# WISDEM/RAFT

Measured on AMD Instinct MI355X. Metric: design-case-frequency solves/sec (whole node), higher is better.
Workload: dtype f64

## Files before the change

### raft_amd/csrc/raftx_geom.h

```cpp
#pragma once

#define MP_N 24
#define MH_N 48
#define MI_N 48

__host__ __device__ inline void derive_design_tables(const double *strips, int64_t i0, int64_t i1, double *dsv,
                                                     int *dsf) {
    int64_t s = i0;
    while (s < i1) {
        int64_t e = s + 1;
        double proj[64];
        int np = 0;
        while (e < i1 && (e - s) < 64) {
            const double *pr = strips + (size_t)(e - 1) * NF, *cr = strips + (size_t)e * NF;
            bool same = true;
            double dv[3], pj = 0.0;
            for (int j = 0; j < 3; j++) {
                same = same && (pr[RAFTX_F_Q + j] == cr[RAFTX_F_Q + j]);
                dv[j] = cr[RAFTX_F_X + j] - pr[RAFTX_F_X + j];
                pj += dv[j] * cr[RAFTX_F_Q + j];
            }
            if (!same || !(pj > 0.0) || !(fabs(pj) <= 1.797e308)) break;
            double perp2 = 0.0, scale = 1.0;
            for (int j = 0; j < 3; j++) {
// ... 79 lines not shown
    double *Ms, *Cs, *Ws;
    const double *Fz;
    double *drho;
    double rho, g;
    int nw;
    const double *k;
    int *cnt, *cntm;
    double *mpose, *mhyd;
    double *abi;
    double *mcfaux;
    cplx *cm;
    int64_t *off, *cmoff;
    double *ds;
    int *dsi;
    double *A, *Ch, *Wh, *props;
    double *M0, *C0;
    int add_mask;
    int addup_in_design;
    long long *tot;
    long long *hostOut;
    int64_t mbase, sbase, cbase;
    int *mdesign_w;
    int mgrid;
    __device__ int64_t mo(int d) const { return memberOff[d] - mbase; }
    __device__ int64_t so(int64_t m) const { return stationOff[m] - sbase; }
    __device__ int64_t co(int64_t m) const { return capOff[m] - cbase; }
};

#define GEOM_NOFMA _Pragma("clang fp contract(off)")

__device__ inline double geom_interp(double x, const double *gs, int n, int f) {
    GEOM_NOFMA
    if (x < gs[RAFTX_GS_S]) return gs[f];
    if (x > gs[(size_t)(n - 1) * RAFTX_GS_N + RAFTX_GS_S]) return gs[(size_t)(n - 1) * RAFTX_GS_N + f];
    int j = 0;
    for (int i = 0; i < n; i++)
        if (gs[(size_t)i * RAFTX_GS_N + RAFTX_GS_S] <= x) j = i;
    const double fj = gs[(size_t)j * RAFTX_GS_N + f];
    if (j == n - 1) return fj;
    const double xj = gs[(size_t)j * RAFTX_GS_N + RAFTX_GS_S];
    if (xj == x) return fj;
    const double slope = (gs[(size_t)(j + 1) * RAFTX_GS_N + f] - fj) / (gs[(size_t)(j + 1) * RAFTX_GS_N + RAFTX_GS_S] - xj);
    return slope * (x - xj) + fj;
}

struct GLocate {
// ... 358 lines not shown
    if (d == 0) { A.off[0] = 0; A.cmoff[0] = 0; }
    if (d < A.nDesign)
        for (int64_t m = A.mo(d); m < A.mo(d + 1); m++) A.mdesign_w[m] = d;
}
#define GEOM_MAX_STATIONS 1024
__device__ inline int64_t geom_member_of_thread(const GeomArgs &A) {
    const int64_t t = (int64_t)blockIdx.x * blockDim.x + threadIdx.x;
    if (A.mgrid <= 0) return t < A.nMember ? t : -1;
    const int64_t k = t / A.nDesign;
    if (k >= A.mgrid) return -1;
    const int d = (int)(t % A.nDesign);
    const int64_t m = A.mo(d) + k;
    return m < A.mo(d + 1) ? m : -1;
}
__device__ __forceinline__ void geom_load_row(const double *gs, int i, double (&r)[RAFTX_GS_N]) {
    const double2 *p = reinterpret_cast<const double2 *>(gs + (size_t)i * RAFTX_GS_N);
#pragma unroll
    for (int k = 0; k < RAFTX_GS_N / 2; k++) {
        const double2 v = p[k];
        r[2 * k] = v.x;
        r[2 * k + 1] = v.y;
    }
}
__global__ __launch_bounds__(128) void k_geom_member(GeomArgs A) {
    GEOM_NOFMA
    if (A.mgrid > 0 && A.err[2]) return;
    const int64_t m = geom_member_of_thread(A);
    if (m < 0) return;
    if (A.err[2]) {
        A.cnt[m] = 0;
        A.cntm[m] = 0;
        return;
    }
    double gm[RAFTX_GM_N];
    {
        const double2 *p = reinterpret_cast<const double2 *>(A.gm + (size_t)m * RAFTX_GM_N);
#pragma unroll
        for (int k = 0; k < RAFTX_GM_N / 2; k++) {
            const double2 v = p[k];
            gm[2 * k] = v.x;
            gm[2 * k + 1] = v.y;
        }
    }
    const int64_t so0 = A.so(m), so1 = A.so(m + 1);
    const int64_t co0 = A.capOff ? A.co(m) : 0, co1 = A.capOff ? A.co(m + 1) : 0;
    const int d = A.mdesign[m];
    const double *gs = A.gs + (size_t)so0 * RAFTX_GS_N;
    const int n = (int)(so1 - so0);
    if (n < 2 || n > GEOM_MAX_STATIONS || !(gm[RAFTX_GM_DLSMAX] > 0.0) || !(gm[RAFTX_GM_L] > 0.0)) {
        A.cnt[m] = 0;
        A.cntm[m] = 0;
        atomicCAS(A.err + 3, 0, (int)(m + 1));
        return;
    }
    if (((int)gm[RAFTX_GM_FLAGS] & RAFTX_GM_FLAG_MCF) && gm[RAFTX_GM_SHAPE] != 0.0 && !A.k) {
        A.cnt[m] = 0;
        A.cntm[m] = 0;
        atomicCAS(A.err + 3, 0, -(int)(m + 1));
        return;
    }
    double ps[6] = {0, 0, 0, 0, 0, 0};
    if (A.pose)
        for (int i = 0; i < 6; i++) ps[i] = A.pose[(size_t)d * 6 + i];
    double a[RAFTX_GS_N], b[RAFTX_GS_N];
    geom_load_row(gs, 0, b);
    const bool circ = gm[RAFTX_GM_SHAPE] != 0.0;
    const int flags = (int)gm[RAFTX_GM_FLAGS];
    double rA0[3], q0[3], nrm = 0.0;
    for (int i = 0; i < 3; i++) {
        rA0[i] = gm[RAFTX_GM_RA + i];
        q0[i] = gm[RAFTX_GM_RB + i] - gm[RAFTX_GM_RA + i];
        nrm += q0[i] * q0[i];
    }
    nrm = sqrt(nrm);
    for (int i = 0; i < 3; i++) q0[i] /= nrm;
    const double beta = atan2(q0[1], q0[0]);
    const double phi = atan2(sqrt(q0[0] * q0[0] + q0[1] * q0[1]), q0[2]);
    const double gam = gm[RAFTX_GM_GAMMA] * (M_PI / 180.0);
    const double s1 = sin(beta), c1 = cos(beta), s2 = sin(phi), c2 = cos(phi), s3 = sin(gam), c3 = cos(gam);
    const double R0[3][3] = {{c1 * c2 * c3 - s1 * s3, -c3 * s1 - c1 * c2 * s3, c1 * s2},
                             {c1 * s3 + c2 * c3 * s1, c1 * c3 - c2 * s1 * s3, s1 * s2},
                             {-c3 * s2, s2 * s3, c2}};
    const double p10[3] = {R0[0][0], R0[1][0], R0[2][0]};
    const double p20[3] = {q0[1] * p10[2] - q0[2] * p10[1], q0[2] * p10[0] - q0[0] * p10[2], q0[0] * p10[1] - q0[1] * p10[0]};
    const double sy = sin(ps[5]), cy = cos(ps[5]), sp = sin(ps[4]), cp = cos(ps[4]), sr = sin(ps[3]), cr = cos(ps[3]);
    const double Rp[3][3] = {{cy * cp, cy * sp * sr - cr * sy, sy * sr + cy * cr * sp},
                             {cp * sy, cy * cr + sy * sp * sr, cr * sy * sp - cy * sr},
                             {-sp, cp * sr, cp * cr}};
    double q[3], p1[3], p2[3], rA[3], rB[3], R[2][2];
    const double L = gm[RAFTX_GM_L];
    for (int i = 0; i < 3; i++) {
        q[i] = Rp[i][0] * q0[0] + Rp[i][1] * q0[1] + Rp[i][2] * q0[2];
        p1[i] = Rp[i][0] * p10[0] + Rp[i][1] * p10[1] + Rp[i][2] * p10[2];
        p2[i] = Rp[i][0] * p20[0] + Rp[i][1] * p20[1] + Rp[i][2] * p20[2];
        const double dsp = (Rp[i][0] - (i == 0 ? 1.0 : 0.0)) * rA0[0] + (Rp[i][1] - (i == 1 ? 1.0 : 0.0)) * rA0[1] +
                           (Rp[i][2] - (i == 2 ? 1.0 : 0.0)) * rA0[2];
        rA[i] = rA0[i] + (ps[i] + dsp);
    }
    for (int i = 0; i < 3; i++) rB[i] = rA[i] + L * q[i];
    for (int i = 0; i < 2; i++)
        for (int j = 0; j < 2; j++) R[i][j] = Rp[i][0] * R0[0][j] + Rp[i][1] * R0[1][j] + Rp[i][2] * R0[2][j];
    int wet = 0;
    if (geom_along(rA[2], rB[2], 0.0, L) < 0) wet++;
    double C[36], F[6], Vt = 0.0, rcV[3] = {0, 0, 0}, AWPm = 0.0;
    for (int i = 0; i < 36; i++) C[i] = 0.0;
    for (int i = 0; i < 6; i++) F[i] = 0.0;
    const double beta2 = atan2(q[1], q[0]), phi2 = atan2(sqrt(q[0] * q[0] + q[1] * q[1]), q[2]);
    const double cosPhi = cos(phi2), sinPhi = sin(phi2), tanPhi = tan(phi2), cosBeta = cos(beta2), sinBeta = sin(beta2);
    const double rg = A.rho * A.g;
    const bool nostatic = (flags & RAFTX_GM_FLAG_NOSTATIC) != 0;
    const double rho_shell = gm[RAFTX_GM_RHOSHELL];
    const bool trim = (A.add_mask & RAFTX_TRIM_BALLAST) != 0;
    for (int i = 1; i < n; i++) {
#pragma unroll
        for (int f = 0; f < RAFTX_GS_N; f++) a[f] = b[f];
        geom_load_row(gs, i, b);
        {
            const double lstrip = b[RAFTX_GS_S] - a[RAFTX_GS_S];
            const int cntg = geom_interval_strips(lstrip, gm[RAFTX_GM_DLSMAX]);
            for (int j = 0; j < cntg; j++) {
                double ls;
                if (lstrip > 0.0) {
                    const double dl = lstrip / cntg;
                    ls = a[RAFTX_GS_S] + dl * (0.5 + j);
                } else {
                    ls = a[RAFTX_GS_S];
                }
                if (geom_along(rA[2], rB[2], ls, L) < 0) wet++;
            }
        }
        if (nostatic) continue;
        {
            double ra[3], rb[3];
            for (int c = 0; c < 3; c++) {
                ra[c] = rA[c] + q[c] * a[RAFTX_GS_S];
// ... 47 lines not shown
                C[4 * 6 + 5] += -rg * V * (rc[1] - rA[1]);
                Vt += V;
                for (int c = 0; c < 3; c++) rcV[c] += rc[c] * V;
                AWPm = AWP;
            } else if (ra[2] <= 0 && rb[2] <= 0) {
                double V, hc;
                geom_frustum(a[RAFTX_GS_D], aD1, b[RAFTX_GS_D], bD1, circ, b[RAFTX_GS_S] - a[RAFTX_GS_S], V, hc);
                double rc[3], rr[3];
                for (int c = 0; c < 3; c++) { rc[c] = ra[c] + q[c] * hc; rr[c] = rc[c] - rA[c]; }
                const double Fz = rg * V;
                F[2] += Fz;
                F[3] += rr[1] * Fz;
                F[4] += -rr[0] * Fz;
                C[3 * 6 + 3] += rg * V * rr[2];
                C[4 * 6 + 4] += rg * V * rr[2];
                C[3 * 6 + 5] += -rg * V * rr[0];
                C[4 * 6 + 5] += -rg * V * rr[1];
                Vt += V;
                for (int c = 0; c < 3; c++) rcV[c] += rc[c] * V;
            }
        }
    }
    if (geom_along(rA[2], rB[2], b[RAFTX_GS_S], L) < 0) wet++;
    double *mh = A.mhyd + (size_t)m * MH_N, *mi = A.minert + (size_t)m * MI_N;
    if (!nostatic) {
        for (int i = 0; i < 36; i++) mh[i] = C[i];
        for (int i = 0; i < 6; i++) mh[36 + i] = F[i];
        mh[42] = Vt; mh[43] = rcV[0]; mh[44] = rcV[1]; mh[45] = rcV[2]; mh[46] = AWPm; mh[47] = 0.0;
    }
    int code = 0;
    if (!nostatic) {
        GInertia J;
        geom_inertia_init(J);
        geom_load_row(gs, 0, b);
        for (int i = 1; i < n; i++) {
#pragma unroll
            for (int f = 0; f < RAFTX_GS_N; f++) a[f] = b[f];
            geom_load_row(gs, i, b);
            geom_inertia_section(J, a, b, circ, rho_shell, trim, 0.0, rA, q, p1, p2);
        }
        const int ncap = A.capOff ? (int)(co1 - co0) : 0;
        const double *gc = A.capOff ? A.caps + (size_t)co0 * RAFTX_GC_N : nullptr;
        code = geom_inertia_caps_finish(J, gs, n, gc, ncap, circ, rho_shell, rA, q, p1, p2, A.g, mi);
    }
    double *mp = A.mpose + (size_t)m * MP_N;
    for (int i = 0; i < 3; i++) {
        mp[i] = rA0[i]; mp[3 + i] = rA[i]; mp[6 + i] = q[i]; mp[9 + i] = p1[i]; mp[12 + i] = p2[i];
    }
    mp[15] = R[0][0]; mp[16] = R[0][1]; mp[17] = R[1][0]; mp[18] = R[1][1]; mp[19] = L;
    const int wetm = ((flags & RAFTX_GM_FLAG_MCF) && circ && !(flags & RAFTX_GM_FLAG_POTMOD)) ? wet : 0;
    A.cnt[m] = wet;
    A.cntm[m] = wetm;
    if (wet) atomicAdd(reinterpret_cast<unsigned long long *>(A.off + d + 1), (unsigned long long)wet);
    if (wetm) atomicAdd(reinterpret_cast<unsigned long long *>(A.cmoff + d + 1), (unsigned long long)wetm);
    if (nostatic) {
        for (int i = 0; i < MH_N; i++) mh[i] = 0.0;
        for (int i = 0; i < MI_N; i++) mi[i] = 0.0;
        return;
    }
    if (code) {
        for (int i = 0; i < MI_N; i++) mi[i] = 0.0;
        atomicCAS(A.err, 0, (int)(m + 1));
    }
}

__global__ void k_geom_trim(GeomArgs A) {
    GEOM_NOFMA
    if (A.err[2] | A.err[3]) return;
    const int d = blockIdx.x * blockDim.x + threadIdx.x;
    if (d >= A.nDesign) return;
    double mass = A.M0[(size_t)d * 36], V = 0.0, vol = 0.0;
    for (int64_t m = A.mo(d); m < A.mo(d + 1); m++) {
        mass += A.minert[(size_t)m * MI_N + 36];
        vol += A.minert[(size_t)m * MI_N + 47];
        V += A.mhyd[(size_t)m * MH_N + 42];
    }
    if (!(vol > 0.0)) {
        A.drho[d] = 0.0;
        atomicCAS(A.err + 1, 0, d + 1);
        return;
    }
    const double sumFz = -mass * A.g + V * A.rho * A.g + (A.Fz ? A.Fz[d] : 0.0);
    A.drho[d] = sumFz / A.g / vol;
}
__global__ __launch_bounds__(128) void k_geom_reinertia(GeomArgs A) {
    GEOM_NOFMA
// ... 184 lines not shown
#endif
static_assert(GD_T % 64 == 0 && GD_T % DS_N == 0 && GD_T <= 256, "k_geom_design: whole wavefronts, a lane keeps its record field");
template <bool ABI, bool ADDUP>
__device__ __forceinline__ void geom_design_block(const GeomArgs &A, const int d, double *gd_lds, int *wcnt) {
    GEOM_NOFMA
    const int lane = threadIdx.x;
    const int64_t i0 = A.off[d], i1 = A.off[d + 1];
    const int S = (int)(i1 - i0);
    double *rec = gd_lds;
    double *pjv = rec + (size_t)S * GD_ROW, *unv = pjv + S;
    int *okv = reinterpret_cast<int *>(unv + S), *rsv = okv + S, *mfl = rsv + S;
    GEOM_PHASE_BEGIN
    {
        const int64_t m0 = A.mo(d), m1 = A.mo(d + 1);
        const int nMem = (int)(m1 - m0);
        const int64_t s0 = A.so(m0);
        const int nSta = (int)(A.so(m1) - s0);
        int *mcum = mfl + S;
        int *mbase = mcum + nSta + 2 * nMem;
        int *ssta = mbase + nMem + 1;
        double *sgm = reinterpret_cast<double *>(okv + (((int)(ssta - okv) + nMem + 2) & ~1));
        double *sgs = sgm + (size_t)nMem * GD_GM_N;
        double *smp = sgs + (size_t)nSta * RAFTX_GS_N;
        {
            const double *g0 = A.gm + (size_t)m0 * RAFTX_GM_N, *g1 = A.gs + (size_t)s0 * RAFTX_GS_N, *g2 = A.mpose + (size_t)m0 * MP_N;
            const int n0 = nMem * GD_GM_N, n01 = n0 + nSta * RAFTX_GS_N, total = n01 + nMem * GD_MP_N;
            constexpr int SU = 10;
            const int64_t so_lane = lane <= nMem ? A.so(m0 + lane) : s0;
            for (int base = 0; base < total; base += SU * GD_T) {
                double v[SU];
#pragma unroll
                for (int u = 0; u < SU; u++) {
                    const int idx = base + u * GD_T + lane;
                    const double *src;
                    if (idx < n0) {
                        const int row = idx / GD_GM_N, col = idx % GD_GM_N;
                        src = g0 + (size_t)row * RAFTX_GM_N + (col == 0 ? RAFTX_GM_DLSMAX : (col == 1 ? RAFTX_GM_SHAPE : RAFTX_GM_FLAGS));
                    } else if (idx < n01) {
                        src = g1 + (idx - n0);
                    } else {
                        const int k = idx - n01, row = k / GD_MP_N, col = k % GD_MP_N;
                        src = g2 + (size_t)row * MP_N + (col < 12 ? 3 + col : 19);
                    }
                    v[u] = idx < total ? *src : 0.0;
                }
#pragma unroll
                for (int u = 0; u < SU; u++) {
                    const int idx = base + u * GD_T + lane;
                    if (idx < total) sgm[idx] = v[u];
                }
            }
            if (lane <= nMem) mbase[lane] = ssta[lane] = (int)(so_lane - s0);
            for (int mi = lane + GD_T; mi <= nMem; mi += GD_T) mbase[mi] = ssta[mi] = (int)(A.so(m0 + mi) - s0);
        }
        __syncthreads();
        for (int u = lane; u < nSta + nMem; u += GD_T) {
            int mi = 0;
            while (mi + 1 < nMem && mbase[mi + 1] + mi + 1 <= u) mi++;
            const int sta0 = mbase[mi], n = mbase[mi + 1] - sta0, g = u - (sta0 + mi);
            int cntg = 1;
            if (g > 0 && g < n) {
                const double *gs = sgs + (size_t)sta0 * RAFTX_GS_N;
                cntg = geom_interval_strips(gs[(size_t)g * RAFTX_GS_N + RAFTX_GS_S] - gs[(size_t)(g - 1) * RAFTX_GS_N + RAFTX_GS_S],
                                            sgm[(size_t)mi * GD_GM_N]);
            }
            mcum[sta0 + 2 * mi + g + 1] = cntg;
        }
        __syncthreads();
        for (int mi = lane; mi < nMem; mi += GD_T) {
            const int n = ssta[mi + 1] - ssta[mi];
            int *cum = mcum + ssta[mi] + 2 * mi;
            int a = 0;
            cum[0] = 0;
            for (int g = 0; g <= n; g++) { a += cum[g + 1]; cum[g + 1] = a; }
            mbase[mi + 1] = a;
        }
        __syncthreads();
        if (lane == 0) {
            int a = 0;
            mbase[0] = 0;
            for (int mi = 0; mi < nMem; mi++) { a += mbase[mi + 1]; mbase[mi + 1] = a; }
        }
        __syncthreads();
        const int total = mbase[nMem];
        GEOM_PHASE(0);
        const double rho = A.rho, cdrag = sqrt(8 / M_PI);
        double rP[3] = {0, 0, 0};
        if (A.pose)
            for (int i = 0; i < 3; i++) rP[i] = A.pose[(size_t)d * 6 + i];
        int nwet = 0;
        for (int t0 = 0; t0 < total; t0 += GD_T) {
            const int t = t0 + lane;
            const bool act = t < total;
            const int tq = act ? t : 0;
            int mi = 0;
            while (mi + 1 < nMem && mbase[mi + 1] <= tq) mi++;
            const int64_t m = m0 + mi;
// ... 469 lines not shown
```

### raft_amd/csrc/raftx_hip.hip

```cpp

#include <hip/hip_runtime.h>
#include <rccl/rccl.h>
#include <dlfcn.h>

#include <algorithm>
#include <cmath>
#include <cstdint>
#include <cstdio>
#include <cstdlib>
#include <cstring>
#include <chrono>
#include <map>
#include <functional>
#include <mutex>
#include <type_traits>
#include <thread>
#include <unordered_map>
#include <vector>

#include "../../include/raftx.h"
#include "../../include/raftx_modal.h"
#include "../../include/raftx_current.h"
#include "../../include/raftx_channels.h"

// ... 635 lines not shown
struct BuildJob {
    GeomArgs A;
    std::vector<void *> tmp;
    int nDesign = 0, nw = 0;
    int64_t maxMem = 0, maxSta = 0;
    size_t nStrips = 0, nRows = 0;
    int maxS = 0;
    double *M0d = nullptr, *C0d = nullptr;
    const double *B0d = nullptr, *MBwd = nullptr;
    bool active = false;
    hipStream_t reduce_stream = nullptr;
    bool gen_deferred = false;
    size_t gen_lds = 0;
};

struct CaseSet {
    std::vector<double> key;
    DevTables T;
    std::vector<void *> allocs;
    int users = 0;
    unsigned long long stamp = 0;
};

struct VariantProg {
    int nM = 0, nSt = 0, nCap = 0, nP = 0;
    bool has_caps = false;
    double *gm = nullptr, *gs = nullptr, *gc = nullptr;
    int *stMember = nullptr, *capMember = nullptr;
    double *stFrac = nullptr, *fillFrac = nullptr, *capFrac = nullptr;
    double *endCoef = nullptr, *headCS = nullptr, *diaCoef = nullptr;
    int *endEdit = nullptr, *diaEdit = nullptr;
    std::vector<int64_t> hS, hC;
    std::vector<void *> allocs;
    int cachedN = -1;
    std::vector<int64_t> memberOff, stationOff, capOff;
};
struct VariantSrc {
    const VariantProg *prog;
    const double *params;
};

static void expand_args(const VariantProg &P, int n, double *gm_out, double *gs_out, double *gc_out, ExpandArgs &E) {
    E.n = n; E.nM = P.nM; E.nSt = P.nSt; E.nCap = P.nCap; E.nP = P.nP;
    E.gm = P.gm; E.gs = P.gs; E.gc = P.gc;
    E.stMember = P.stMember; E.capMember = P.capMember;
    E.stFrac = P.stFrac; E.fillFrac = P.fillFrac; E.capFrac = P.capFrac;
    E.endCoef = P.endCoef; E.headCS = P.headCS; E.diaCoef = P.diaCoef;
    E.endEdit = P.endEdit; E.diaEdit = P.diaEdit;
    E.gm_out = gm_out; E.gs_out = gs_out; E.gc_out = gc_out;
}

struct DenseResident {
    int nSet = 0, n = 0, nw = 0, freq_mask = 0;
    double *w = nullptr, *M = nullptr, *B = nullptr, *C = nullptr;
    std::vector<void *> allocs;
};
struct raftx_ctx {
    int device;
    hipStream_t stream;
    bool owns_stream;
    hipEvent_t ev0, ev1;
    hipEvent_t evUp, evTot, evG0, evG1, evG2, evG3, evS0, evS1, evDone;
// ... 66 lines not shown
    int comm_rank, comm_world;
    int *commFlag = nullptr;
    std::vector<raftx_ctx *> workers[RAFTX_NSLOT];
    struct SweepSlot *slots;
    VariantProg vprog;
};
struct DevOffsets {
    const int64_t *memberOff, *stationOff, *capOff;
};
struct SeaStates { int nCase, nHead, nw; const double *w, *k; double depth, rho, g; const double *zeta, *beta; };
struct BuildSource {
    const int64_t *memberOff, *stationOff, *capOff;
    const double *members, *stations, *caps;
    const double *pose, *M0, *B0, *C0, *MBw, *Fz_moor, *k;
    double rho, g;
    int nw, add_mask;
    DevOffsets dOff{nullptr, nullptr, nullptr};
    const double *k_dev = nullptr;
    VariantSrc var{nullptr, nullptr};
};
struct SweepSlot {
    bool busy = false;
    int cset = -1;
    bool prepared = false;
    int nIter = 0;
    double tol = 0, XiStart = 0, dw = 0;
    std::vector<raftx_ctx *> blk;
    std::vector<int> bnd;
    int nCase = 0, nHead = 0, nw = 0;
    double *sd = nullptr;
    int32_t *niter = nullptr, *flags = nullptr;
    raftx_c128 *Xi = nullptr;
    int64_t *stripOffsets = nullptr;
    std::vector<void *> allocs;
    hipEvent_t evXi = nullptr;
    BuildSource p1;
    size_t next_p1 = 0;
    std::chrono::steady_clock::time_point t0;
    double since() const { return std::chrono::duration<double, std::milli>(std::chrono::steady_clock::now() - t0).count(); }
    double tl[4] = {0, 0, 0, 0};
    double span[2] = {0, 0};
    size_t nSlabEv = 0;
    bool slab = false;
    std::vector<double> tlb;
    struct {
        bool on = false;
// ... 95 lines not shown
    c->comm_world = 1;
    c->owns_stream = true;
    c->slots = new SweepSlot[RAFTX_NSLOT];
    c->sCopy = c->sPrep = c->sD2H = c->sGen = nullptr;
    bool ok = hipStreamCreateWithFlags(&c->stream, hipStreamNonBlocking) == hipSuccess;
    c->sAux = nullptr;
    for (hipEvent_t *e : {&c->evZ, &c->ev0, &c->ev1, &c->evUp, &c->evTot, &c->evG0, &c->evG1, &c->evG2, &c->evG3, &c->evS0,
                          &c->evS1, &c->evDone, &c->evMem, &c->evRed})
        ok = ok && hipEventCreate(e) == hipSuccess;
    if (!ok) {
        delete[] c->slots;
        delete c;
        return -6;
    }
    *out = c;
    return 0;
}

static void free_list(raftx_ctx *c, std::vector<void *> &v) {
    for (void *p : v) c->pool.put(p);
    v.clear();
}

extern "C" void raftx_ctx_destroy(raftx_ctx *c) {
    if (!c) return;
#ifdef GEOM_PHASE_TIMING
    if (c->owns_stream && c->slots) {
        unsigned long long ph[10] = {0};
        (void)hipDeviceSynchronize();
        if (hipMemcpyFromSymbol(ph, HIP_SYMBOL(geom_phase_cycles), sizeof(ph)) == hipSuccess && ph[0]) {
            unsigned long long tot = 0;
            for (int i = 0; i < 7; i++) tot += ph[i];
            fprintf(stderr, "[k_geom_design phases, %% of wave time] counts %.1f | generate %.1f | abi out %.1f | runs %.1f | ds out %.1f | g-vectors %.1f | morison+matrices %.1f\n",
                    100.0 * ph[0] / tot, 100.0 * ph[1] / tot, 100.0 * ph[2] / tot, 100.0 * ph[3] / tot, 100.0 * ph[4] / tot,
                    100.0 * ph[5] / tot, 100.0 * ph[6] / tot);
        }
    }
#endif
    (void)raftx_comm_destroy(c);
    if (c->owns_stream) {
        (void)hipSetDevice(c->device);
        (void)hipDeviceSynchronize();
    }
    for (int sl = 0; sl < RAFTX_NSLOT; sl++) {
        for (raftx_ctx *w : c->workers[sl]) raftx_ctx_destroy(w);
        c->workers[sl].clear();
    }
    (void)hipSetDevice(c->device);
    (void)hipStreamSynchronize(c->stream);
    free_list(c, c->design_allocs);
    free_list(c, c->case_allocs);
    free_list(c, c->result_allocs);
    for (CaseSet &cs : c->csets) free_list(c, cs.allocs);
    c->pool.trim();
    if (c->rXl) (void)hipFree(c->rXl);
    if (c->rXlSlots) (void)hipFree(c->rXlSlots);
    if (c->kpCtr) (void)hipFree(c->kpCtr);
    if (c->flexXl0) (void)hipFree(c->flexXl0);
    if (c->rXl0) (void)hipFree(c->rXl0);
    if (c->rXlOut) (void)hipFree(c->rXlOut);
    if (c->rQtf) (void)hipFree(c->rQtf);
    if (c->bemF) (void)hipFree(c->bemF);
    if (c->rKay) (void)hipFree(c->rKay);
    if (c->pairList) (void)hipFree(c->pairList);
    free_list(c, c->dense.allocs);
    free_list(c, c->vprog.allocs);
    if (c->identList) (void)hipFree(c->identList);
    for (hipEvent_t e : c->evSlab) (void)hipEventDestroy(e);
    if (c->evFork) (void)hipEventDestroy(c->evFork);
    if (c->evJoin) (void)hipEventDestroy(c->evJoin);
    free_list(c, c->job.tmp);
    for (int sl = 0; sl < RAFTX_NSLOT; sl++) {
        free_list(c, c->slots[sl].allocs);
        if (c->slots[sl].evXi) (void)hipEventDestroy(c->slots[sl].evXi);
        if (c->slots[sl].modal.evUp) (void)hipEventDestroy(c->slots[sl].modal.evUp);
        if (c->slots[sl].current.evUp) (void)hipEventDestroy(c->slots[sl].current.evUp);
        if (c->slots[sl].channels.evUp) (void)hipEventDestroy(c->slots[sl].channels.evUp);
    }
    delete[] c->slots;
    c->pool.trim();
    c->pin.release();
    c->pinRes.release();
    c->pinModal.release();
    c->pinCur.release();
    c->pinChan.release();
    for (hipEvent_t e : {c->evZ, c->ev0, c->ev1, c->evUp, c->evTot, c->evG0, c->evG1, c->evG2, c->evG3, c->evS0, c->evS1, c->evDone,
                         c->evMem, c->evRed})
        (void)hipEventDestroy(e);
    if (c->sAux) (void)hipStreamDestroy(c->sAux);
// ... 255 lines not shown
    RangeScope range_("build phase 1: descriptor H2D, member pass, scans (enqueue)");
    BuildJob &J = c->job;
    Slice L;
    if (int rc = slice_of(c, B, lo, nDesign, L)) return rc;
    HIPCHK(c, hipSetDevice(c->device));
    free_list(c, c->design_allocs);
    free_list(c, J.tmp);
    c->have_designs = false; c->bem_ready = false; c->g_n = 0;
    HIPCHK(c, c->pin.reserve(PIN_OFF + (size_t)nDesign + 1));
    GeomArgs &A = J.A;
    memset(&A, 0, sizeof(A));
    A.nDesign = nDesign; A.nMember = L.m1 - L.m0;
    A.rho = B.rho; A.g = B.g; A.nw = B.nw; A.add_mask = B.add_mask;
    A.mbase = L.m0; A.sbase = L.s0; A.cbase = L.c0;
    A.hostOut = c->pin.p;
    memset(c->pin.p, 0, (PIN_OFF + 1) * sizeof(long long));
    J.nDesign = nDesign; J.nw = B.nw;
    ExpandArgs E;
    if (int rc = upload_descriptors(c, sCopy, B, L, E)) return rc;
    HIPCHK(c, hipEventRecord(c->evUp, sCopy));
    HIPCHK(c, hipStreamWaitEvent(sPrep, c->evUp, 0));
    if (B.var.prog && nDesign > 0) {
        launch_expand(E, sPrep);
    }
    if (int rc = alloc_member_scratch(c)) return rc;
    if (int rc = design_bounds(c, B, L)) return rc;
    if (int rc = enqueue_member_pass(c, sPrep)) return rc;
    if (int rc = enqueue_scan_reduce(c, sPrep)) return rc;
    J.active = true;
    return 0;
}

constexpr int GEN_CROSSING = 1;
constexpr int GEN_MAY_DEFER = 2;
constexpr int GEN_PIPELINED = 4;
static void launch_design(raftx_ctx *c, hipStream_t st) {
    hipLaunchKernelGGL(k_geom_design, dim3((unsigned)c->job.nDesign), dim3(GD_T), c->job.gen_lds, st, c->job.A);
}
static int wait_totals(raftx_ctx *c, int64_t *stripOffsets) {
    BuildJob &J = c->job;
    for (;;) {
        const hipError_t q = hipEventQuery(c->evTot);
        if (q == hipSuccess) break;
        if (q != hipErrorNotReady) HIPCHK(c, q);
    }
    HIPCHK(c, hipGetLastError());
// ... 1598 lines not shown
    double tot = 0;
    for (double v : fr) tot += v;
    std::vector<int> b{0};
    double acc = 0;
    for (size_t i = 0; i < fr.size(); i++) {
        acc += fr[i];
        int hi = (i + 1 == fr.size()) ? nDesign : (int)llround(acc / tot * nDesign);
        if (hi > nDesign) hi = nDesign;
        if (hi > b.back()) b.push_back(hi);
    }
    if (b.back() != nDesign) b.push_back(nDesign);
    return b;
}

static bool others_in_flight(raftx_ctx *c, int slot) {
    for (int sl = 0; sl < RAFTX_NSLOT; sl++)
        if (sl != slot && (c->slots[sl].busy || c->slots[sl].prepared)) return true;
    return false;
}

static void slot_release_cases(raftx_ctx *c, SweepSlot &S) {
    if (S.cset >= 0 && c->csets[S.cset].users > 0) c->csets[S.cset].users--;
    S.cset = -1;
}

static int sweep_fail_drain(raftx_ctx *c, SweepSlot &S, int rc) {
    (void)hipDeviceSynchronize();
    for (raftx_ctx *sub : S.blk)
        if (sub) build_abandon(sub);
    slot_release_cases(c, S);
    return rc;
}

static int crossing_streams(raftx_ctx *c, SweepSlot &S) {
    if (!c->sCopy) {
        HIPCHK(c, hipStreamCreateWithFlags(&c->sCopy, hipStreamNonBlocking));
        HIPCHK(c, hipStreamCreateWithFlags(&c->sPrep, hipStreamNonBlocking));
        HIPCHK(c, hipStreamCreateWithFlags(&c->sD2H, hipStreamNonBlocking));
        HIPCHK(c, hipStreamCreateWithFlags(&c->sGen, hipStreamNonBlocking));
    }
    if (!S.evXi) HIPCHK(c, hipEventCreate(&S.evXi));
    return 0;
}
static int acquire_cases(raftx_ctx *c, SweepSlot &S, const SeaStates &sea) {
    const int nCase = sea.nCase, nHead = sea.nHead, nw = sea.nw;
    std::vector<double> key;
// ... 33 lines not shown
    S.dw = sea.nw > 1 ? sea.w[1] - sea.w[0] : sea.w[0];
    S.nIter = run.nIter; S.tol = run.tol; S.XiStart = run.XiStart;
    S.blk.assign(S.bnd.size() - 1, nullptr);
    S.nCase = sea.nCase; S.nHead = sea.nHead; S.nw = sea.nw;
    S.sd = run.sd; S.niter = run.niter; S.flags = run.flags; S.Xi = run.Xi; S.stripOffsets = run.stripOffsets;
    S.tl[0] = S.since();
    free_list(c, S.allocs);
    S.modal.on = S.current.on = S.channels.on = false;
}
static int upload_offsets(raftx_ctx *c, SweepSlot &S, const BuildSource &src, int nDesign) {
    S.p1 = src;
    S.p1.k_dev = c->csets[S.cset].T.k;
    const int64_t nMemberAll = src.memberOff[nDesign];
    DevOffsets &dOff = S.p1.dOff;
    int rc = upload_on(c, c->sCopy, S.allocs, src.memberOff, (size_t)nDesign + 1, &dOff.memberOff);
    rc |= upload_on(c, c->sCopy, S.allocs, src.stationOff, (size_t)nMemberAll + 1, &dOff.stationOff);
    if (src.capOff) rc |= upload_on(c, c->sCopy, S.allocs, src.capOff, (size_t)nMemberAll + 1, &dOff.capOff);
    return rc ? -2 : 0;
}
static int block_phase1(raftx_ctx *c, SweepSlot &S, size_t b) {
    return build_phase1(S.blk[b], c->sCopy, c->sPrep, S.p1, S.bnd[b], S.bnd[b + 1] - S.bnd[b]);
}

static int sweep_prepare_impl(raftx_ctx *c, int slot, int nDesign, const BuildSource &src, const SeaStates &sea, const SweepRun &run) {
    RangeScope range_("raftx_sweep_prepare: descriptor H2D + member pass (enqueue)");
    if (!c) return -1;
    SLOT_REF(S, c, slot, "sweep_prepare");
    if (S.busy || S.prepared) FAIL(c, "sweep_prepare: slot %d is still in flight (call raftx_sweep_wait first)", slot);
    if (int rc = check_source(c, src, nDesign, "sweep_stats", "bad design arguments")) return rc;
    if (sea.nCase < 1 || sea.nHead < 1 || sea.nw < 1 || !sea.w || !sea.k || !sea.zeta || !sea.beta) FAIL(c, "sweep_stats: bad sea-state arguments");
    if (!run.sd || !run.niter || !run.flags) FAIL(c, "sweep_stats: std, niter and flags are required");
    if (run.nIter < 0) FAIL(c, "sweep_stats: nIter < 0");
    HIPCHK(c, hipSetDevice(c->device));
    S.t0 = std::chrono::steady_clock::now();
    if (int rc = crossing_streams(c, S)) return rc;
    if (sea.nw > MAX_NW) FAIL(c, "nw=%d exceeds the %d bins per workgroup supported by this build", sea.nw, MAX_NW);
    if (int rc = acquire_cases(c, S, sea)) return rc;
    cut_blocks(c, slot, nDesign, sea, run);
    if (src.memberOff[nDesign] < 0) {
        slot_release_cases(c, S);
        FAIL(c, "sweep_stats: member offsets not monotone");
    }
    if (int rc = upload_offsets(c, S, src, nDesign)) return sweep_fail_drain(c, S, rc);
    const size_t nB = S.blk.size(), nFirst = (run.Xi && nB > 2 && !others_in_flight(c, slot)) ? 2 : nB;
    for (size_t b = 0; b < nB; b++)
        if (block_ctx(c, slot, b, &S.blk[b])) return sweep_fail_drain(c, S, -1);
    for (size_t b = 0; b < nFirst; b++)
        if (const int rc = block_phase1(c, S, b)) {
            snprintf(c->err, sizeof(c->err), "sweep_stats (block %zu): %s", b, S.blk[b]->err);
            return sweep_fail_drain(c, S, rc);
        }
    S.next_p1 = nFirst;
    S.tl[1] = S.since();
    S.prepared = true;
    return 0;
}

extern "C" int raftx_sweep_prepare(raftx_ctx *c, int slot, int nDesign, const int64_t *memberOff, const double *members,
                                  const int64_t *stationOff, const double *stations, const int64_t *capOff,
                                  const double *caps, const double *pose, double rho, double g, int add_mask,
                                  const double *M0, const double *B0, const double *C0, const double *Fz_moor, int nCase,
                                  int nHead, int nw, const double *w, const double *k, double depth, double rho_wave,
                                  double g_wave, const double *zeta, const double *beta, int nIter, double tol,
                                  double XiStart, int nChunk, double *sd, int32_t *niter, int32_t *flags,
                                  raftx_c128 *Xi, int64_t *stripOffsets) {
    const BuildSource src{memberOff, stationOff, capOff, members, stations, caps, pose, M0, B0, C0, nullptr, Fz_moor, k, rho, g, nw, add_mask};
    return sweep_prepare_impl(c, slot, nDesign, src, SeaStates{nCase, nHead, nw, w, k, depth, rho_wave, g_wave, zeta, beta},
                              SweepRun{nIter, tol, XiStart, nChunk, sd, niter, flags, Xi, stripOffsets});
}

extern "C" int raftx_variant_program(raftx_ctx *c, int nMember, const double *members, const int64_t *stationOff, const double *stations,
                                     const int64_t *capOff, const double *caps, int nParam, const double *endCoef,
                                     const int32_t *endEdit, const double *headCS, const double *diaCoef, const int32_t *diaEdit) {
    if (!c) return -1;
    for (int sl = 0; sl < RAFTX_NSLOT; sl++)
        if (c->slots && (c->slots[sl].busy || c->slots[sl].prepared) && c->slots[sl].p1.var.prog)
            FAIL(c, "variant_program: a batch of variants is still in flight (raftx_sweep_wait first)");
    HIPCHK(c, hipSetDevice(c->device));
    HIPCHK(c, hipStreamSynchronize(c->stream));
    VariantProg &P = c->vprog;
    free_list(c, P.allocs);
    P = VariantProg();
    if (nMember == 0) return 0;
    if (nMember < 0 || nParam < 0 || nParam > 64 || !members || !stationOff || !stations || (capOff == nullptr) != (caps == nullptr))
        FAIL(c, "variant_program: bad arguments");
    if (!endEdit || !endCoef || !headCS || !diaEdit || !diaCoef) FAIL(c, "variant_program: the edit tables are required (all-zero flags = no edit)");
    const int nM = nMember, nP = nParam;
    if (stationOff[0] != 0 || (capOff && capOff[0] != 0)) FAIL(c, "variant_program: offsets must start at 0");
    for (int m = 0; m < nM; m++)
        if (stationOff[m + 1] < stationOff[m] || (capOff && capOff[m + 1] < capOff[m])) FAIL(c, "variant_program: offsets not monotone");
    const int nSt = (int)stationOff[nM], nCap = capOff ? (int)capOff[nM] : 0;
    std::vector<int> stM((size_t)nSt), cpM((size_t)nCap);
    std::vector<double> stF((size_t)nSt), flF((size_t)nSt), cpF((size_t)nCap);
    for (int m = 0; m < nM; m++) {
        const double L = members[(size_t)m * RAFTX_GM_N + RAFTX_GM_L];
        if (endEdit[m] && !(L > 0.0)) FAIL(c, "variant_program: member %d has no length", m);
        for (int64_t i = stationOff[m]; i < stationOff[m + 1]; i++) {
            stM[(size_t)i] = m;
            stF[(size_t)i] = stations[(size_t)i * RAFTX_GS_N + RAFTX_GS_S] / L;
            flF[(size_t)i] = stations[(size_t)i * RAFTX_GS_N + RAFTX_GS_LFILL] / L;
        }
        if (capOff)
            for (int64_t i = capOff[m]; i < capOff[m + 1]; i++) {
                cpM[(size_t)i] = m;
                cpF[(size_t)i] = caps[(size_t)i * RAFTX_GC_N + RAFTX_GC_S] / L;
// ... 5 lines not shown
    else P.hC.assign((size_t)nM + 1, 0);
    auto up = [&](const void *h, size_t bytes, void **d) -> int {
        *d = nullptr;
        if (!bytes) bytes = 8, h = nullptr;
        HIPCHK(c, hipMalloc(d, bytes));
        P.allocs.push_back(*d);
        if (h) HIPCHK(c, hipMemcpy(*d, h, bytes, hipMemcpyHostToDevice));
        return 0;
    };
    int rc = 0;
    rc |= up(members, (size_t)nM * RAFTX_GM_N * 8, (void **)&P.gm);
    rc |= up(stations, (size_t)nSt * RAFTX_GS_N * 8, (void **)&P.gs);
    rc |= up(nCap ? caps : nullptr, (size_t)nCap * RAFTX_GC_N * 8, (void **)&P.gc);
    rc |= up(stM.data(), (size_t)nSt * 4, (void **)&P.stMember);
    rc |= up(nCap ? cpM.data() : nullptr, (size_t)nCap * 4, (void **)&P.capMember);
    rc |= up(stF.data(), (size_t)nSt * 8, (void **)&P.stFrac);
    rc |= up(flF.data(), (size_t)nSt * 8, (void **)&P.fillFrac);
    rc |= up(nCap ? cpF.data() : nullptr, (size_t)nCap * 8, (void **)&P.capFrac);
    rc |= up(endCoef, (size_t)nM * 6 * (nP + 1) * 8, (void **)&P.endCoef);
    rc |= up(headCS, (size_t)nM * 2 * 8, (void **)&P.headCS);
    rc |= up(diaCoef, (size_t)nSt * 2 * (nP + 1) * 8, (void **)&P.diaCoef);
    rc |= up(endEdit, (size_t)nM * 4, (void **)&P.endEdit);
    rc |= up(diaEdit, (size_t)nSt * 4, (void **)&P.diaEdit);
    if (rc) {
        free_list(c, P.allocs);
        P = VariantProg();
        return rc;
    }
    return 0;
}
static void variant_offsets(VariantProg &P, int n) {
    if (P.cachedN == n) return;
    P.memberOff.resize((size_t)n + 1);
    P.stationOff.resize((size_t)n * P.nM + 1);
    P.capOff.resize((size_t)n * P.nM + 1);
    for (int d = 0; d <= n; d++) P.memberOff[(size_t)d] = (int64_t)d * P.nM;
    for (int d = 0; d < n; d++)
        for (int m = 0; m < P.nM; m++) {
            P.stationOff[(size_t)d * P.nM + m] = (int64_t)d * P.nSt + P.hS[(size_t)m];
            P.capOff[(size_t)d * P.nM + m] = (int64_t)d * P.nCap + P.hC[(size_t)m];
        }
    P.stationOff[(size_t)n * P.nM] = (int64_t)n * P.nSt;
    P.capOff[(size_t)n * P.nM] = (int64_t)n * P.nCap;
    P.cachedN = n;
}
extern "C" int raftx_expand_variants(raftx_ctx *c, int nDesign, const double *params, double *members, double *stations, double *caps) {
    if (!c) return -1;
    const VariantProg &P = c->vprog;
    if (!P.nM) FAIL(c, "expand_variants: no program (raftx_variant_program first)");
    if (nDesign < 0 || (!params && nDesign && P.nP) || !members || !stations) FAIL(c, "expand_variants: bad arguments");
    if (!nDesign) return 0;
// ... 961 lines not shown
```

Before: 677.5 million.

## Precompute geometry of unedited members once and copy cached records per design

Members whose ends and diameters are never edited by the variant program now have their geometry (pose, hydrostatics, inertia and wet-strip counts) computed once per (rho, g, trim, haveK) setting by a new kernel. The result is stored in per-slot records that are reference-counted and event-synchronised. The per-design member kernel then copies these records instead of recomputing the body, so per-design work covers only edited members. A separate change zeroes strip prefix sums for members with no wet strips. The cost is more device memory, more slot and event bookkeeping, and a risk of stale records if the cache key misses a relevant input.

Result: faster. 687.2 million, median of 6 (+1.4%).

```diff
diff --git a/raft_amd/csrc/raftx_geom.h b/raft_amd/csrc/raftx_geom.h
--- a/raft_amd/csrc/raftx_geom.h
+++ b/raft_amd/csrc/raftx_geom.h
@@ -125,6 +125,9 @@
     int64_t mbase, sbase, cbase;
     int *mdesign_w;
     int mgrid;
+    const double *fixRec;
+    const int *fixInt, *fixIdx;
+    int fixNM;
     __device__ int64_t mo(int d) const { return memberOff[d] - mbase; }
     __device__ int64_t so(int64_t m) const { return stationOff[m] - sbase; }
     __device__ int64_t co(int64_t m) const { return capOff[m] - cbase; }
@@ -529,19 +532,21 @@
         r[2 * k + 1] = v.y;
     }
 }
-__global__ __launch_bounds__(128) void k_geom_member(GeomArgs A) {
-    GEOM_NOFMA
-    if (A.mgrid > 0 && A.err[2]) return;
-    const int64_t m = geom_member_of_thread(A);
-    if (m < 0) return;
-    if (A.err[2]) {
-        A.cnt[m] = 0;
-        A.cntm[m] = 0;
-        return;
-    }
+struct GMember {
+    int wet, wetm;
+    int code;
+    int rej;
+};
+#define FR_N (MP_N + MH_N + MI_N)
+#define FR_I 4
+__device__ __forceinline__ GMember geom_member_body(const double *gmrow, const double *gs, const int n, const double *gc, const int ncap,
+                                                    const double *pose, const double rho, const double g, const bool trim,
+                                                    const bool haveK, double *mp, double *mh, double *mi) {
+    GEOM_NOFMA
+    GMember res = {0, 0, 0, 0};
     double gm[RAFTX_GM_N];
     {
-        const double2 *p = reinterpret_cast<const double2 *>(A.gm + (size_t)m * RAFTX_GM_N);
+        const double2 *p = reinterpret_cast<const double2 *>(gmrow);
 #pragma unroll
         for (int k = 0; k < RAFTX_GM_N / 2; k++) {
             const double2 v = p[k];
@@ -549,26 +554,17 @@
             gm[2 * k + 1] = v.y;
         }
     }
-    const int64_t so0 = A.so(m), so1 = A.so(m + 1);
-    const int64_t co0 = A.capOff ? A.co(m) : 0, co1 = A.capOff ? A.co(m + 1) : 0;
-    const int d = A.mdesign[m];
-    const double *gs = A.gs + (size_t)so0 * RAFTX_GS_N;
-    const int n = (int)(so1 - so0);
     if (n < 2 || n > GEOM_MAX_STATIONS || !(gm[RAFTX_GM_DLSMAX] > 0.0) || !(gm[RAFTX_GM_L] > 0.0)) {
-        A.cnt[m] = 0;
-        A.cntm[m] = 0;
-        atomicCAS(A.err + 3, 0, (int)(m + 1));
-        return;
-    }
-    if (((int)gm[RAFTX_GM_FLAGS] & RAFTX_GM_FLAG_MCF) && gm[RAFTX_GM_SHAPE] != 0.0 && !A.k) {
-        A.cnt[m] = 0;
-        A.cntm[m] = 0;
-        atomicCAS(A.err + 3, 0, -(int)(m + 1));
-        return;
+        res.rej = 1;
+        return res;
+    }
+    if (((int)gm[RAFTX_GM_FLAGS] & RAFTX_GM_FLAG_MCF) && gm[RAFTX_GM_SHAPE] != 0.0 && !haveK) {
+        res.rej = 2;
+        return res;
     }
     double ps[6] = {0, 0, 0, 0, 0, 0};
-    if (A.pose)
-        for (int i = 0; i < 6; i++) ps[i] = A.pose[(size_t)d * 6 + i];
+    if (pose)
+        for (int i = 0; i < 6; i++) ps[i] = pose[i];
     double a[RAFTX_GS_N], b[RAFTX_GS_N];
     geom_load_row(gs, 0, b);
     const bool circ = gm[RAFTX_GM_SHAPE] != 0.0;
@@ -614,10 +610,9 @@
     for (int i = 0; i < 6; i++) F[i] = 0.0;
     const double beta2 = atan2(q[1], q[0]), phi2 = atan2(sqrt(q[0] * q[0] + q[1] * q[1]), q[2]);
     const double cosPhi = cos(phi2), sinPhi = sin(phi2), tanPhi = tan(phi2), cosBeta = cos(beta2), sinBeta = sin(beta2);
-    const double rg = A.rho * A.g;
+    const double rg = rho * g;
     const bool nostatic = (flags & RAFTX_GM_FLAG_NOSTATIC) != 0;
     const double rho_shell = gm[RAFTX_GM_RHOSHELL];
-    const bool trim = (A.add_mask & RAFTX_TRIM_BALLAST) != 0;
     for (int i = 1; i < n; i++) {
 #pragma unroll
         for (int f = 0; f < RAFTX_GS_N; f++) a[f] = b[f];
@@ -711,7 +706,6 @@
         }
     }
     if (geom_along(rA[2], rB[2], b[RAFTX_GS_S], L) < 0) wet++;
-    double *mh = A.mhyd + (size_t)m * MH_N, *mi = A.minert + (size_t)m * MI_N;
     if (!nostatic) {
         for (int i = 0; i < 36; i++) mh[i] = C[i];
         for (int i = 0; i < 6; i++) mh[36 + i] = F[i];
@@ -728,29 +722,95 @@
             geom_load_row(gs, i, b);
             geom_inertia_section(J, a, b, circ, rho_shell, trim, 0.0, rA, q, p1, p2);
         }
-        const int ncap = A.capOff ? (int)(co1 - co0) : 0;
-        const double *gc = A.capOff ? A.caps + (size_t)co0 * RAFTX_GC_N : nullptr;
-        code = geom_inertia_caps_finish(J, gs, n, gc, ncap, circ, rho_shell, rA, q, p1, p2, A.g, mi);
-    }
-    double *mp = A.mpose + (size_t)m * MP_N;
+        code = geom_inertia_caps_finish(J, gs, n, gc, ncap, circ, rho_shell, rA, q, p1, p2, g, mi);
+    }
     for (int i = 0; i < 3; i++) {
         mp[i] = rA0[i]; mp[3 + i] = rA[i]; mp[6 + i] = q[i]; mp[9 + i] = p1[i]; mp[12 + i] = p2[i];
     }
     mp[15] = R[0][0]; mp[16] = R[0][1]; mp[17] = R[1][0]; mp[18] = R[1][1]; mp[19] = L;
     const int wetm = ((flags & RAFTX_GM_FLAG_MCF) && circ && !(flags & RAFTX_GM_FLAG_POTMOD)) ? wet : 0;
-    A.cnt[m] = wet;
-    A.cntm[m] = wetm;
-    if (wet) atomicAdd(reinterpret_cast<unsigned long long *>(A.off + d + 1), (unsigned long long)wet);
-    if (wetm) atomicAdd(reinterpret_cast<unsigned long long *>(A.cmoff + d + 1), (unsigned long long)wetm);
+    res.wet = wet;
+    res.wetm = wetm;
     if (nostatic) {
         for (int i = 0; i < MH_N; i++) mh[i] = 0.0;
         for (int i = 0; i < MI_N; i++) mi[i] = 0.0;
-        return;
+        return res;
     }
     if (code) {
         for (int i = 0; i < MI_N; i++) mi[i] = 0.0;
-        atomicCAS(A.err, 0, (int)(m + 1));
-    }
+        res.code = code;
+    }
+    return res;
+}
+
+struct FixedArgs {
+    int nFix;
+    const double *gm, *gs, *gc;
+    const int *desc;
+    double rho, g;
+    int trim, haveK;
+    double *rec;
+    int *irec;
+};
+__global__ __launch_bounds__(64) void k_geom_member_fixed(FixedArgs F) {
+    const int f = blockIdx.x * blockDim.x + threadIdx.x;
+    if (f >= F.nFix) return;
+    const int *ds = F.desc + (size_t)f * 5;
+    double *r = F.rec + (size_t)f * FR_N;
+    const GMember R = geom_member_body(F.gm + (size_t)ds[0] * RAFTX_GM_N, F.gs + (size_t)ds[1] * RAFTX_GS_N, ds[2],
+                                       ds[4] >= 0 ? F.gc + (size_t)ds[3] * RAFTX_GC_N : nullptr, ds[4] >= 0 ? ds[4] : 0, nullptr, F.rho,
+                                       F.g, F.trim != 0, F.haveK != 0, r, r + MP_N, r + MP_N + MH_N);
+    int *ir = F.irec + (size_t)f * FR_I;
+    ir[0] = R.wet; ir[1] = R.wetm; ir[2] = R.code; ir[3] = R.rej;
+}
+__global__ __launch_bounds__(128) void k_geom_member(GeomArgs A) {
+    GEOM_NOFMA
+    if (A.mgrid > 0 && A.err[2]) return;
+    const int64_t m = geom_member_of_thread(A);
+    if (m < 0) return;
+    if (A.err[2]) {
+        A.cnt[m] = 0;
+        A.cntm[m] = 0;
+        return;
+    }
+    GMember R;
+    int d;
+    const int fix = A.fixRec ? A.fixIdx[m % A.fixNM] : -1;
+    if (fix >= 0) {
+        d = (int)(m / A.fixNM);
+        const int4 ir = *reinterpret_cast<const int4 *>(A.fixInt + (size_t)fix * FR_I);
+        R.wet = ir.x; R.wetm = ir.y; R.code = ir.z; R.rej = ir.w;
+        if (!R.rej) {
+            const double2 *src = reinterpret_cast<const double2 *>(A.fixRec + (size_t)fix * FR_N);
+            double2 *mp = reinterpret_cast<double2 *>(A.mpose + (size_t)m * MP_N), *mh = reinterpret_cast<double2 *>(A.mhyd + (size_t)m * MH_N),
+                    *mi = reinterpret_cast<double2 *>(A.minert + (size_t)m * MI_N);
+#pragma unroll
+            for (int i = 0; i < MP_N / 2; i++) mp[i] = src[i];
+#pragma unroll 8
+            for (int i = 0; i < MH_N / 2; i++) mh[i] = src[MP_N / 2 + i];
+#pragma unroll 8
+            for (int i = 0; i < MI_N / 2; i++) mi[i] = src[(MP_N + MH_N) / 2 + i];
+        }
+    } else {
+        const int64_t so0 = A.so(m), so1 = A.so(m + 1);
+        const int64_t co0 = A.capOff ? A.co(m) : 0, co1 = A.capOff ? A.co(m + 1) : 0;
+        d = A.mdesign[m];
+        R = geom_member_body(A.gm + (size_t)m * RAFTX_GM_N, A.gs + (size_t)so0 * RAFTX_GS_N, (int)(so1 - so0),
+                             A.capOff ? A.caps + (size_t)co0 * RAFTX_GC_N : nullptr, A.capOff ? (int)(co1 - co0) : 0,
+                             A.pose ? A.pose + (size_t)d * 6 : nullptr, A.rho, A.g, (A.add_mask & RAFTX_TRIM_BALLAST) != 0, A.k != nullptr,
+                             A.mpose + (size_t)m * MP_N, A.mhyd + (size_t)m * MH_N, A.minert + (size_t)m * MI_N);
+    }
+    if (R.rej) {
+        A.cnt[m] = 0;
+        A.cntm[m] = 0;
+        atomicCAS(A.err + 3, 0, R.rej == 1 ? (int)(m + 1) : -(int)(m + 1));
+        return;
+    }
+    A.cnt[m] = R.wet;
+    A.cntm[m] = R.wetm;
+    if (R.wet) atomicAdd(reinterpret_cast<unsigned long long *>(A.off + d + 1), (unsigned long long)R.wet);
+    if (R.wetm) atomicAdd(reinterpret_cast<unsigned long long *>(A.cmoff + d + 1), (unsigned long long)R.wetm);
+    if (R.code) atomicCAS(A.err, 0, (int)(m + 1));
 }
 
 __global__ void k_geom_trim(GeomArgs A) {
@@ -981,11 +1041,13 @@
         double *sgm = reinterpret_cast<double *>(okv + (((int)(ssta - okv) + nMem + 2) & ~1));
         double *sgs = sgm + (size_t)nMem * GD_GM_N;
         double *smp = sgs + (size_t)nSta * RAFTX_GS_N;
+        int cnt_lane = 0;
         {
             const double *g0 = A.gm + (size_t)m0 * RAFTX_GM_N, *g1 = A.gs + (size_t)s0 * RAFTX_GS_N, *g2 = A.mpose + (size_t)m0 * MP_N;
             const int n0 = nMem * GD_GM_N, n01 = n0 + nSta * RAFTX_GS_N, total = n01 + nMem * GD_MP_N;
             constexpr int SU = 10;
             const int64_t so_lane = lane <= nMem ? A.so(m0 + lane) : s0;
+            cnt_lane = lane < nMem ? A.cnt[m0 + lane] : 0;
             for (int base = 0; base < total; base += SU * GD_T) {
                 double v[SU];
 #pragma unroll
@@ -1029,9 +1091,10 @@
         for (int mi = lane; mi < nMem; mi += GD_T) {
             const int n = ssta[mi + 1] - ssta[mi];
             int *cum = mcum + ssta[mi] + 2 * mi;
+            const bool dry = (mi == lane ? cnt_lane : A.cnt[m0 + mi]) == 0;
             int a = 0;
             cum[0] = 0;
-            for (int g = 0; g <= n; g++) { a += cum[g + 1]; cum[g + 1] = a; }
+            for (int g = 0; g <= n; g++) { a += dry ? 0 : cum[g + 1]; cum[g + 1] = a; }
             mbase[mi + 1] = a;
         }
         __syncthreads();
diff --git a/raft_amd/csrc/raftx_hip.hip b/raft_amd/csrc/raftx_hip.hip
--- a/raft_amd/csrc/raftx_hip.hip
+++ b/raft_amd/csrc/raftx_hip.hip
@@ -681,8 +681,23 @@
     unsigned long long stamp = 0;
 };
 
+struct FixedRecord {
+    bool valid = false;
+    double rho = 0, g = 0;
+    int trim = 0, haveK = 0;
+    double *rec = nullptr;
+    int *irec = nullptr;
+    int users = 0;
+    unsigned long long stamp = 0;
+    hipEvent_t ev = nullptr;
+    hipStream_t stream = nullptr;
+};
 struct VariantProg {
     int nM = 0, nSt = 0, nCap = 0, nP = 0;
+    int nFix = 0;
+    int *fixDesc = nullptr, *fixIdx = nullptr;
+    FixedRecord recs[RAFTX_NSLOT + 1];
+    unsigned long long rec_clock = 0;
     bool has_caps = false;
     double *gm = nullptr, *gs = nullptr, *gc = nullptr;
     int *stMember = nullptr, *capMember = nullptr;
@@ -697,6 +712,7 @@
 struct VariantSrc {
     const VariantProg *prog;
     const double *params;
+    const FixedRecord *rec = nullptr;
 };
 
 static void expand_args(const VariantProg &P, int n, double *gm_out, double *gs_out, double *gc_out, ExpandArgs &E) {
@@ -809,6 +825,7 @@
 struct SweepSlot {
     bool busy = false;
     int cset = -1;
+    int frec = -1;
     bool prepared = false;
     int nIter = 0;
     double tol = 0, XiStart = 0, dw = 0;
@@ -950,6 +967,12 @@
     v.clear();
 }
 
+static void variant_release(raftx_ctx *c) {
+    for (FixedRecord &R : c->vprog.recs)
+        if (R.ev) (void)hipEventDestroy(R.ev);
+    free_list(c, c->vprog.allocs);
+    c->vprog = VariantProg();
+}
 extern "C" void raftx_ctx_destroy(raftx_ctx *c) {
     if (!c) return;
 #ifdef GEOM_PHASE_TIMING
@@ -992,7 +1015,7 @@
     if (c->rKay) (void)hipFree(c->rKay);
     if (c->pairList) (void)hipFree(c->pairList);
     free_list(c, c->dense.allocs);
-    free_list(c, c->vprog.allocs);
+    variant_release(c);
     if (c->identList) (void)hipFree(c->identList);
     for (hipEvent_t e : c->evSlab) (void)hipEventDestroy(e);
     if (c->evFork) (void)hipEventDestroy(c->evFork);
@@ -1294,6 +1317,10 @@
     HIPCHK(c, hipStreamWaitEvent(sPrep, c->evUp, 0));
     if (B.var.prog && nDesign > 0) {
         launch_expand(E, sPrep);
+        if (const FixedRecord *R = B.var.rec) {
+            if (R->stream != sPrep) HIPCHK(c, hipStreamWaitEvent(sPrep, R->ev, 0));
+            A.fixRec = R->rec; A.fixInt = R->irec; A.fixIdx = B.var.prog->fixIdx; A.fixNM = B.var.prog->nM;
+        }
     }
     if (int rc = alloc_member_scratch(c)) return rc;
     if (int rc = design_bounds(c, B, L)) return rc;
@@ -2938,6 +2965,8 @@
 static void slot_release_cases(raftx_ctx *c, SweepSlot &S) {
     if (S.cset >= 0 && c->csets[S.cset].users > 0) c->csets[S.cset].users--;
     S.cset = -1;
+    if (S.frec >= 0 && c->vprog.recs[S.frec].users > 0) c->vprog.recs[S.frec].users--;
+    S.frec = -1;
 }
 
 static int sweep_fail_drain(raftx_ctx *c, SweepSlot &S, int rc) {
@@ -3017,6 +3046,7 @@
     return build_phase1(S.blk[b], c->sCopy, c->sPrep, S.p1, S.bnd[b], S.bnd[b + 1] - S.bnd[b]);
 }
 
+static int acquire_fixed(raftx_ctx *c, SweepSlot &S);
 static int sweep_prepare_impl(raftx_ctx *c, int slot, int nDesign, const BuildSource &src, const SeaStates &sea, const SweepRun &run) {
     RangeScope range_("raftx_sweep_prepare: descriptor H2D + member pass (enqueue)");
     if (!c) return -1;
@@ -3037,6 +3067,7 @@
         FAIL(c, "sweep_stats: member offsets not monotone");
     }
     if (int rc = upload_offsets(c, S, src, nDesign)) return sweep_fail_drain(c, S, rc);
+    if (int rc = acquire_fixed(c, S)) return sweep_fail_drain(c, S, rc);
     const size_t nB = S.blk.size(), nFirst = (run.Xi && nB > 2 && !others_in_flight(c, slot)) ? 2 : nB;
     for (size_t b = 0; b < nB; b++)
         if (block_ctx(c, slot, b, &S.blk[b])) return sweep_fail_drain(c, S, -1);
@@ -3074,8 +3105,7 @@
     HIPCHK(c, hipSetDevice(c->device));
     HIPCHK(c, hipStreamSynchronize(c->stream));
     VariantProg &P = c->vprog;
-    free_list(c, P.allocs);
-    P = VariantProg();
+    variant_release(c);
     if (nMember == 0) return 0;
     if (nMember < 0 || nParam < 0 || nParam > 64 || !members || !stationOff || !stations || (capOff == nullptr) != (caps == nullptr))
         FAIL(c, "variant_program: bad arguments");
@@ -3127,11 +3157,60 @@
     rc |= up(diaCoef, (size_t)nSt * 2 * (nP + 1) * 8, (void **)&P.diaCoef);
     rc |= up(endEdit, (size_t)nM * 4, (void **)&P.endEdit);
     rc |= up(diaEdit, (size_t)nSt * 4, (void **)&P.diaEdit);
+    std::vector<int> desc, fidx((size_t)nM, -1);
+    for (int m = 0; m < nM; m++) {
+        bool fixed = endEdit[m] == 0;
+        for (int64_t i = stationOff[m]; fixed && i < stationOff[m + 1]; i++) fixed = diaEdit[i] == 0;
+        if (!fixed) continue;
+        fidx[(size_t)m] = P.nFix++;
+        desc.insert(desc.end(), {m, (int)stationOff[m], (int)(stationOff[m + 1] - stationOff[m]), capOff ? (int)capOff[m] : 0,
+                                 capOff ? (int)(capOff[m + 1] - capOff[m]) : -1});
+    }
+    if (P.nFix) {
+        rc |= up(desc.data(), desc.size() * 4, (void **)&P.fixDesc);
+        rc |= up(fidx.data(), (size_t)nM * 4, (void **)&P.fixIdx);
+        for (FixedRecord &R : P.recs) {
+            rc |= up(nullptr, (size_t)P.nFix * FR_N * 8, (void **)&R.rec);
+            rc |= up(nullptr, (size_t)P.nFix * FR_I * 4, (void **)&R.irec);
+            if (!rc) HIPCHK(c, hipMemset(R.rec, 0, (size_t)P.nFix * FR_N * 8));
+        }
+    }
     if (rc) {
-        free_list(c, P.allocs);
-        P = VariantProg();
+        variant_release(c);
         return rc;
     }
+    return 0;
+}
+static int acquire_fixed(raftx_ctx *c, SweepSlot &S) {
+    VariantProg &P = c->vprog;
+    BuildSource &src = S.p1;
+    src.var.rec = nullptr;
+    if (src.var.prog != &P || !P.nFix || src.pose) return 0;
+    const int trim = (src.add_mask & RAFTX_TRIM_BALLAST) != 0, haveK = src.k_dev != nullptr;
+    int hit = -1, idle = -1;
+    for (int i = 0; i <= RAFTX_NSLOT; i++) {
+        const FixedRecord &R = P.recs[i];
+        if (R.valid && R.rho == src.rho && R.g == src.g && R.trim == trim && R.haveK == haveK) hit = i;
+        else if (R.users == 0 && (idle < 0 || R.stamp < P.recs[idle].stamp)) idle = i;
+    }
+    if (hit < 0) {
+        if (idle < 0) FAIL(c, "sweep_prepare_variants: no free record of the fixed members");
+        FixedRecord &R = P.recs[idle];
+        R.valid = false;
+        if (!R.ev) HIPCHK(c, hipEventCreateWithFlags(&R.ev, hipEventDisableTiming));
+        FixedArgs F{P.nFix, P.gm, P.gs, P.gc, P.fixDesc, src.rho, src.g, trim, haveK, R.rec, R.irec};
+        hipLaunchKernelGGL(k_geom_member_fixed, dim3((unsigned)((P.nFix + 63) / 64)), dim3(64), 0, c->sPrep, F);
+        HIPCHK(c, hipGetLastError());
+        HIPCHK(c, hipEventRecord(R.ev, c->sPrep));
+        R.stream = c->sPrep;
+        R.rho = src.rho; R.g = src.g; R.trim = trim; R.haveK = haveK;
+        R.valid = true;
+        hit = idle;
+    }
+    P.recs[hit].users++;
+    P.recs[hit].stamp = ++P.rec_clock;
+    S.frec = hit;
+    src.var.rec = &P.recs[hit];
     return 0;
 }
 static void variant_offsets(VariantProg &P, int n) {
```
